# vision-agh/apse_uav

Hardware: AMD Instinct MI355X
Metric: 4K UAV frames/sec (whole node) (higher is better)
Workload: dtype f32

## Files before the change

### apse_uav_amd/_lib.py

```python
import ctypes as C
import os

import numpy as np

_HERE = os.path.dirname(os.path.abspath(__file__))
LIB_PATH = os.environ.get("APSE_HIP_LIB") or os.path.join(_HERE, "libapse_hip.so")

APSE_OK = 0


class ApseError(RuntimeError):
    pass


class Config(C.Structure):
    _fields_ = [
        ("struct_size", C.c_int), ("device", C.c_int), ("max_batch", C.c_int),
        ("frame_h", C.c_int), ("frame_w", C.c_int), ("image_h", C.c_int), ("image_w", C.c_int),
        ("blocks", C.c_int * 4), ("num_classes", C.c_int),
        ("score_thresh", C.c_float), ("box_nms", C.c_float), ("rpn_nms", C.c_float), ("mask_thresh", C.c_float),
        ("rpn_pre_topk", C.c_int), ("rpn_post_topk", C.c_int), ("dets_per_image", C.c_int),
        ("pixel_mean", C.c_float * 3), ("assoc_roi", C.c_int), ("embed_dim", C.c_int), ("assoc_scale", C.c_float),
        ("compute_dtype", C.c_int), ("storage16", C.c_int),
    ]


class ConfigArch(Config):
    _fields_ = [("arch", C.c_int)]


class ResultsLayout(C.Structure):
    _fields_ = [("bytes", C.c_size_t), ("n_max", C.c_int), ("dets_per_image", C.c_int), ("embed_dim", C.c_int),
                ("max_batch", C.c_int)] + [(k, C.c_size_t) for k in (
                    "total", "offset", "prop_count", "img", "cls", "roi", "score", "box_resized", "box", "valid", "rect",
                    "mass", "centroid", "closest", "embedding")]


class RenderItem(C.Structure):
    _fields_ = [("image", C.c_int), ("rect", C.c_int * 4), ("words_per_row", C.c_int), ("bits", C.c_void_p),
                ("box", C.c_float * 4), ("rgb", C.c_uint8 * 4), ("label_off", C.c_int), ("label_len", C.c_int)]


class MotsWindow(C.Structure):
    _fields_ = [("rect", C.c_int * 4), ("words_per_row", C.c_int), ("area", C.c_int), ("bits", C.c_void_p)]


class MotsObject(C.Structure):
    _fields_ = [("rect", C.c_int * 4), ("words_per_row", C.c_int), ("score", C.c_float), ("bits", C.c_void_p)]


class ConvDesc(C.Structure):
    _fields_ = [(k, C.c_int) for k in ("B", "H", "W", "Cin", "Cout", "KH", "KW", "stride", "pad", "relu", "res_mode",
                                       "cfg", "splitk", "prec", "fuse_reduce", "x_st", "res_st", "y_st")]


_lib = None


def load():
    global _lib
    if _lib is not None:
        return _lib
    if not os.path.exists(LIB_PATH):
        raise ApseError("libapse_hip.so not found at %s: build it with `python -c 'import __graft_entry__ as g; g.build()'` "
                        "or `make -C apse_uav_amd/csrc` (there is no CPU fallback)" % LIB_PATH)
    import torch
    lib = C.CDLL(LIB_PATH)
    vp, i, f, sz = C.c_void_p, C.c_int, C.c_float, C.c_size_t
    sig = {
        "apse_create": ([C.POINTER(Config), C.POINTER(vp)], i),
        "apse_destroy": ([vp], None),
        "apse_last_error": ([vp], C.c_char_p),
        "apse_version": ([], C.c_char_p),
        "apse_set_weight": ([vp, C.c_char_p, vp, C.POINTER(C.c_int64), i], i),
        "apse_finalize_weights": ([vp], i),
        "apse_set_resize_tables": ([vp, vp, vp, i, vp, vp, i], i),
        "apse_set_camera": ([vp, C.POINTER(C.c_double), C.POINTER(C.c_double), i, vp, i, i], i),
        "apse_preprocess_frames": ([vp, vp, i, vp], i),
        "apse_preprocess_images": ([vp, vp, i, vp], i),
        "apse_backbone": ([vp, i, vp], i),
        "apse_rpn": ([vp, i, vp], i),
        "apse_rpn_levels": ([vp, i, i, vp], i),
        "apse_box_head": ([vp, i, vp], i),
        "apse_set_detections": ([vp, vp, vp, vp, vp, i, vp], i),
        "apse_mask_tail": ([vp, i, vp], i),
        "apse_embed": ([vp, i, vp], i),
        "apse_forward": ([vp, i, vp], i),
        "apse_results_describe": ([vp, C.POINTER(ResultsLayout)], i),
        "apse_read_results": ([vp, vp, sz, vp], i),
        "apse_read_results_begin": ([vp, vp, sz, vp], i),
        "apse_read_results_end": ([vp, vp], i),
        "apse_copy_mask_window": ([vp, i, i, i, i, i, vp, vp], i),
        "apse_copy_mask_windows": ([vp, i, vp, vp, vp, vp, vp], i),
        "apse_host_copy": ([vp, vp, sz, i], i),
        "apse_feature_shape": ([vp, C.c_char_p, C.POINTER(C.c_int * 3)], i),
        "apse_export_feature": ([vp, C.c_char_p, vp, i, vp], i),
        "apse_debug_tensor": ([vp, C.c_char_p, vp, sz, C.POINTER(sz), vp], i),
        "apse_flops": ([vp, i, C.c_double, C.c_double], C.c_double),
        "apse_profile": ([vp, i], i),
        "apse_profile_read": ([vp, C.POINTER(C.c_double * 42), i], i),
        "apse_conv_packed_elems": ([C.POINTER(ConvDesc)], sz),
        "apse_conv_pack_weight": ([C.POINTER(ConvDesc), vp, i, vp, vp], i),
        "apse_conv2d": ([C.POINTER(ConvDesc), vp, vp, vp, vp, vp, vp, sz, vp], i),
        "apse_maxpool3x3s2": ([vp, vp, i, i, i, i, vp], i),
        "apse_maxpool3x3s2_typed": ([vp, vp, i, i, i, i, i, vp], i),
        "apse_roi_align": ([C.POINTER(vp), C.POINTER(i), C.POINTER(i), vp, i, i, i, vp, vp], i),
        "apse_roi_align_typed": ([C.POINTER(vp), C.POINTER(i), C.POINTER(i), vp, i, i, i, i, vp, vp], i),
        "apse_roi_pool": ([vp, i, i, vp, vp, i, i, f, vp, vp], i),
        "apse_roi_features": ([vp, i, vp, vp, i, i, vp, vp], i),
        "apse_nms_rank": ([vp, vp, vp, i, i, i, i, f, i, vp, vp, vp, vp, vp], i),
        "apse_mask_centroid_dense": ([vp, i, i, C.POINTER(C.c_int * 3), vp], i),
        "apse_mask_closest_dense": ([vp, i, i, f, f, C.POINTER(C.c_int * 2), vp], i),
        "apse_l2_normalize": ([vp, vp, i, i, vp], i),
        "apse_sqdist": ([vp, vp, i, i, i, vp, vp], i),
        "apse_undistort_gamma": ([vp, vp, i, i, i, C.POINTER(C.c_double), C.POINTER(C.c_double), i, vp, i, i, vp], i),
        "apse_lab_tables_host": ([vp, vp, C.c_size_t], C.c_size_t),
        "apse_replay_create": ([i, i, f, i], vp),
        "apse_replay_destroy": ([vp], None),
        "apse_replay_step": ([vp, i, i, vp, vp, vp, C.c_char_p, i, vp], i),
        "apse_replay_packed": ([vp, vp, C.c_longlong, i, i, i, vp, C.c_longlong], C.c_longlong),
        "apse_replay_max_id": ([vp], i),
        "apse_replay_next_id": ([vp], i),
        "apse_render_workspace_bytes": ([i, i, i], sz),
        "apse_render_instances": ([vp, vp, i, i, i, i, vp, i, vp, sz, vp, i, vp, sz, vp], i),
        "apse_render_pack_mask": ([vp, i, i, vp, vp], i),
        "apse_render_font_host": ([vp, sz], sz),
        "apse_mots_split_workspace_bytes": ([], sz),
        "apse_mots_split_idmap": ([vp, i, i, i, vp, sz, vp, vp, vp, vp, sz, vp], i),
        "apse_mots_rle_to_bits": ([vp, vp, i, i, i, vp, vp], i),
        "apse_mots_overlaps": ([vp, i, vp, i, vp, i, vp, vp], i),
        "apse_mots_render_idmap": ([vp, vp, i, i, i, vp, vp], i),
        "apse_resize_normalize": ([vp, vp, vp, vp, vp, vp, i, vp, vp, i, i, i, i, i, i, i, i, C.POINTER(f * 3), vp], i),
        "apse_assoc_fc_workspace_bytes": ([i, i, i], sz),
        "apse_assoc_fc_forward": ([vp, vp, vp, i, i, i, vp, vp, vp, sz, vp], i),
        "apse_assoc_fc_backward": ([vp, vp, vp, vp, i, i, i, vp, vp, vp, sz, vp], i),
        "apse_triplet_workspace_bytes": ([i], sz),
        "apse_triplet_hard_forward": ([vp, vp, i, i, f, i, vp, vp, sz, vp], i),
        "apse_triplet_all_forward": ([vp, vp, i, i, f, i, vp, vp, sz, vp], i),
        "apse_triplet_hard_backward": ([vp, i, i, i, vp, vp, vp, vp], i),
        "apse_triplet_all_backward": ([vp, i, i, i, vp, vp, vp, vp], i),
        "apse_sgd_step": ([vp, vp, vp, C.c_longlong, f, f, f, f, i, i, vp], i),
        "apse_coco_box_iou": ([vp, vp, vp, i, i, i, vp, vp, vp, vp, vp], i),
        "apse_coco_poly_to_bits": ([vp, vp, i, vp, i, vp, vp, vp, i, vp, vp, vp, vp], i),
        "apse_coco_match": ([vp, vp, vp, i, i, i, vp, vp, vp, i, vp, vp, vp, i, vp, i, vp, i, vp, vp, vp, vp, vp], i),
        "apse_coco_accumulate_workspace_bytes": ([C.c_longlong], sz),
        "apse_coco_sort_lists": ([vp, vp, i, vp, C.c_longlong, i, vp, vp, sz, vp], i),
        "apse_coco_accumulate": ([vp, vp, vp, i, vp, i, vp, vp, vp, C.c_longlong, i, vp, i, i, i, i, i, vp, vp, vp, vp, sz,
                                  vp], i),
        "apse_mask_roi_features": ([vp, i, vp, i, vp, vp], i),
        "apse_mask_train_workspace_bytes": ([i, i], sz),
        "apse_mask_pack_elems": ([i, i, i, i], sz),
        "apse_mask_pack_weight": ([vp, vp, i, i, i, i, i, vp, vp, vp], i),
        "apse_mask_conv_forward": ([vp, vp, vp, i, i, i, i, i, i, i, i, i, i, i, vp, vp, sz, vp], i),
        "apse_mask_conv3x3": ([vp, vp, vp, i, i, vp, vp], i),
        "apse_mask_relu_grad": ([vp, vp, C.c_longlong, vp, vp], i),
        "apse_mask_bias_grad": ([vp, C.c_longlong, vp, vp, sz, vp], i),
        "apse_mask_wgrad": ([vp, vp, i, i, vp, vp, sz, vp], i),
        "apse_mask_loss_forward": ([vp, i, vp, vp, i, vp, vp, sz, vp], i),
        "apse_mask_loss_backward": ([vp, i, vp, vp, i, vp, vp, vp], i),
        "apse_mask_predictor_backward": ([vp, vp, vp, vp, i, i, vp, vp, vp, vp, sz, vp], i),
    }
    for name, (args, ret) in sig.items():
        fn = getattr(lib, name)
        fn.argtypes = args
        fn.restype = ret
    _lib = lib
    return lib


EXPORTS = ["apse_create", "apse_destroy", "apse_last_error", "apse_version", "apse_set_weight", "apse_finalize_weights",
           "apse_set_resize_tables", "apse_set_camera", "apse_preprocess_frames", "apse_preprocess_images", "apse_backbone", "apse_rpn", "apse_rpn_levels",
           "apse_box_head", "apse_set_detections", "apse_mask_tail", "apse_embed", "apse_forward", "apse_results_describe",
           "apse_read_results", "apse_read_results_begin", "apse_read_results_end", "apse_copy_mask_window", "apse_copy_mask_windows", "apse_host_copy", "apse_feature_shape", "apse_export_feature", "apse_debug_tensor",
           "apse_flops", "apse_profile", "apse_profile_read", "apse_conv_packed_elems", "apse_conv_pack_weight", "apse_conv2d", "apse_maxpool3x3s2",
           "apse_maxpool3x3s2_typed", "apse_roi_align", "apse_roi_align_typed", "apse_roi_pool", "apse_roi_features", "apse_nms_rank", "apse_mask_centroid_dense", "apse_mask_closest_dense",
           "apse_l2_normalize", "apse_sqdist", "apse_undistort_gamma", "apse_lab_tables_host", "apse_resize_normalize", "apse_replay_create", "apse_replay_destroy",
           "apse_replay_step", "apse_replay_packed", "apse_replay_max_id", "apse_replay_next_id", "apse_render_workspace_bytes",
           "apse_render_instances", "apse_render_pack_mask", "apse_render_font_host", "apse_mots_split_workspace_bytes",
           "apse_mots_split_idmap", "apse_mots_rle_to_bits", "apse_mots_overlaps", "apse_mots_render_idmap",
           "apse_assoc_fc_workspace_bytes", "apse_assoc_fc_forward", "apse_assoc_fc_backward", "apse_triplet_workspace_bytes",
           "apse_triplet_hard_forward", "apse_triplet_all_forward", "apse_triplet_hard_backward", "apse_triplet_all_backward",
           "apse_sgd_step", "apse_coco_box_iou", "apse_coco_poly_to_bits", "apse_coco_match",
           "apse_coco_accumulate_workspace_bytes", "apse_coco_sort_lists", "apse_coco_accumulate",
           "apse_mask_roi_features", "apse_mask_train_workspace_bytes", "apse_mask_pack_elems", "apse_mask_pack_weight",
           "apse_mask_conv_forward", "apse_mask_conv3x3", "apse_mask_relu_grad", "apse_mask_bias_grad", "apse_mask_wgrad", "apse_mask_loss_forward",
           "apse_mask_loss_backward", "apse_mask_predictor_backward"]


def stream_ptr():
    import torch
    return C.c_void_p(torch.cuda.current_stream().cuda_stream)


def check(rc, ctx=None, what=""):
    if rc != APSE_OK:
        msg = load().apse_last_error(ctx).decode() if ctx is not None else ""
        raise ApseError("%s failed (code %d) %s" % (what, rc, msg))


def ptr(t):
    if t is None:
        return C.c_void_p(0)
    if isinstance(t, np.ndarray):
        assert t.flags["C_CONTIGUOUS"]
        return C.c_void_p(t.ctypes.data)
    assert t.is_contiguous()
    return C.c_void_p(t.data_ptr())
```

### apse_uav_amd/csrc/conv_winograd.hip

```cpp
#include "apse_common.h"

namespace {
constexpr int WTR = 16, WTC = 4;
constexpr int WT = WTR * WTC;
constexpr int WN = 64;
constexpr int KC = 8;
constexpr int NTHR = 512;
constexpr int SLICE_F = 16 * WT * KC;
constexpr size_t WINO_LDS = (size_t)2 * 2 * SLICE_F * sizeof(float);
static_assert(WN == WT, "V and U slices share one size");
static_assert((size_t)16 * WT * 32 * sizeof(float) <= WINO_LDS, "epilogue chunk must fit the staging LDS");
}

__global__ __launch_bounds__(NTHR) void conv_winograd_f32(const ConvParams p) {
    extern __shared__ __attribute__((aligned(16))) char smem[];
    float* Vs = reinterpret_cast<float*>(smem);
    float* Us = Vs + 2 * SLICE_F;
    float* Cs = reinterpret_cast<float*>(smem);

    const int tid = threadIdx.x;
    const int lane = tid & 63, wave = tid >> 6;
    const int fr = lane & 31, fh = lane >> 5;

    const int tiles_y = (p.OH + 2 * WTR - 1) / (2 * WTR), tiles_x = (p.OW + 2 * WTC - 1) / (2 * WTC);
    const int nblk = p.Cout / WN;
    const int nwg = p.B * tiles_y * tiles_x * nblk;
    int bid;
    {
        const int wg = blockIdx.x;
        const int q = nwg >> 3, r = nwg & 7, xcd = wg & 7, idx = wg >> 3;
        bid = (xcd < r ? xcd * (q + 1) : r * (q + 1) + (xcd - r) * q) + idx;
    }
    const int nb = bid % nblk;
    int rest = bid / nblk;
    const int bx = rest % tiles_x; rest /= tiles_x;
    const int by = rest % tiles_y;
    const int b = rest / tiles_y;
    const int oy0 = by * 2 * WTR, ox0 = bx * 2 * WTC, n0 = nb * WN;
    const int C = 1 << p.cin_log2;
    const int nsteps = C / KC;

    const int cg = tid & 1, t = (tid >> 1) & (WT - 1), ti = tid >> 7;
    const int ra = ti == 0 ? 0 : (ti == 2 ? 2 : 1);
    const int rb = ti == 0 ? 2 : (ti == 1 ? 2 : (ti == 2 ? 1 : 3));
    const int iy_a = oy0 + 2 * (t / WTC) - 1 + ra, iy_b = oy0 + 2 * (t / WTC) - 1 + rb;
    const int ix0 = ox0 + 2 * (t % WTC) - 1;
    const __amdgpu_buffer_rsrc_t xrsrc =
        __builtin_amdgcn_make_buffer_rsrc(const_cast<float*>(p.x), 0, (int)((((unsigned)(p.B * p.H * p.W)) << p.cin_log2) * 4u), 0x00020000);
    unsigned xoff[2][4];
#pragma unroll
    for (int r = 0; r < 2; ++r) {
        const int iy = r ? iy_b : iy_a;
#pragma unroll
        for (int c = 0; c < 4; ++c) {
            const int ix = ix0 + c;
            const bool in = (unsigned)iy < (unsigned)p.H && (unsigned)ix < (unsigned)p.W;
            xoff[r][c] = in ? ((((unsigned)((b * p.H + iy) * p.W + ix)) << p.cin_log2) + (unsigned)(cg * 4)) * 4u : 0x80000000u;
        }
    }
    const float* ubase = p.wu + (size_t)n0 * KC;
    const size_t ustep = (size_t)16 * p.Cout * KC;

    f32x4 xr[2][4], ur[4];
    auto fetch = [&](int s) {
        const unsigned kb = (unsigned)(s * KC * 4);
#pragma unroll
        for (int r = 0; r < 2; ++r)
#pragma unroll
            for (int c = 0; c < 4; ++c)
                xr[r][c] = __builtin_bit_cast(f32x4, __builtin_amdgcn_raw_buffer_load_b128(xrsrc, (int)(xoff[r][c] + kb), 0, 0));
        const float* us = ubase + (size_t)s * ustep;
#pragma unroll
        for (int k = 0; k < 4; ++k) {
            const int q = tid + NTHR * k;
            const int xi = q >> 7, co = (q >> 1) & 63, h = q & 1;
            ur[k] = *reinterpret_cast<const f32x4*>(us + ((size_t)xi * p.Cout + co) * KC + h * 4);
        }
    };
    auto stage = [&](int buf) {
        f32x4 x[4];
#pragma unroll
        for (int c = 0; c < 4; ++c) x[c] = ti == 1 ? xr[0][c] + xr[1][c] : xr[0][c] - xr[1][c];
        const f32x4 v[4] = {x[0] - x[2], x[1] + x[2], x[2] - x[1], x[1] - x[3]};
        const int sw = (cg ^ ((t >> 3) & 1)) * 4;
#pragma unroll
        for (int j = 0; j < 4; ++j)
            *reinterpret_cast<f32x4*>(Vs + buf * SLICE_F + ((4 * ti + j) * WT + t) * KC + sw) = v[j];
#pragma unroll
        for (int k = 0; k < 4; ++k) {
            const int q = tid + NTHR * k;
            const int xi = q >> 7, co = (q >> 1) & 63, h = q & 1;
            *reinterpret_cast<f32x4*>(Us + buf * SLICE_F + (xi * WN + co) * KC + ((h ^ ((co >> 3) & 1)) * 4)) = ur[k];
        }
    };

    f32x16 acc[2][2][2];
#pragma unroll
    for (int a = 0; a < 2; ++a)
#pragma unroll
        for (int i = 0; i < 2; ++i)
#pragma unroll
            for (int j = 0; j < 2; ++j)
#pragma unroll
                for (int v = 0; v < 16; ++v) acc[a][i][j][v] = 0.f;

    fetch(0);
    stage(0);
    __syncthreads();
    const int fsw = (fh ^ ((fr >> 3) & 1)) * 4;
    for (int s = 0; s < nsteps; ++s) {
        const int buf = s & 1;
        const bool more = s + 1 < nsteps;
        if (more) fetch(s + 1);
#pragma unroll
        for (int a = 0; a < 2; ++a) {
            const int xi = 2 * wave + a;
            f32x4 af[2], bf[2];
#pragma unroll
            for (int i = 0; i < 2; ++i) af[i] = *reinterpret_cast<const f32x4*>(Vs + buf * SLICE_F + (xi * WT + 32 * i + fr) * KC + fsw);
#pragma unroll
            for (int j = 0; j < 2; ++j) bf[j] = *reinterpret_cast<const f32x4*>(Us + buf * SLICE_F + (xi * WN + 32 * j + fr) * KC + fsw);
#pragma unroll
            for (int k = 0; k < 4; ++k)
#pragma unroll
                for (int i = 0; i < 2; ++i)
#pragma unroll
                    for (int j = 0; j < 2; ++j)
                        acc[a][i][j] = __builtin_amdgcn_mfma_f32_32x32x2f32(af[i][k], bf[j][k], acc[a][i][j], 0, 0, 0);
        }
        if (more) stage(buf ^ 1);
        __syncthreads();
    }

    const int et = tid >> 3, eg = tid & 7;
    const int oy = oy0 + 2 * (et / WTC), ox = ox0 + 2 * (et % WTC);
    typedef unsigned u32x4_t __attribute__((ext_vector_type(4)));
#pragma unroll
    for (int j = 0; j < 2; ++j) {
#pragma unroll
        for (int a = 0; a < 2; ++a)
#pragma unroll
            for (int i = 0; i < 2; ++i)
#pragma unroll
                for (int v = 0; v < 16; ++v) {
                    const int row = 32 * i + (v & 3) + 8 * (v >> 2) + 4 * fh;
                    Cs[((2 * wave + a) * WT + row) * 32 + fr] = acc[a][i][j][v];
                }
        __syncthreads();
        f32x4 m[16];
#pragma unroll
        for (int k = 0; k < 16; ++k) m[k] = *reinterpret_cast<const f32x4*>(Cs + (k * WT + et) * 32 + eg * 4);
        f32x4 s0[4], s1[4];
#pragma unroll
        for (int c = 0; c < 4; ++c) {
            s0[c] = m[c] + m[4 + c] + m[8 + c];
            s1[c] = m[4 + c] - m[8 + c] - m[12 + c];
        }
        const int co = n0 + 32 * j + 4 * eg;
        const f32x4 bias4 = p.bias ? *reinterpret_cast<const f32x4*>(p.bias + co) : f32x4{0.f, 0.f, 0.f, 0.f};
        f32x4 y[2][2] = {{s0[0] + s0[1] + s0[2], s0[1] - s0[2] - s0[3]}, {s1[0] + s1[1] + s1[2], s1[1] - s1[2] - s1[3]}};
#pragma unroll
        for (int dy = 0; dy < 2; ++dy)
#pragma unroll
            for (int dx = 0; dx < 2; ++dx) {
                f32x4 val = y[dy][dx] + bias4;
                if (p.relu) {
#pragma unroll
                    for (int k = 0; k < 4; ++k) val[k] = apse_relu(val[k]);
                }
                if (oy + dy < p.OH && ox + dx < p.OW)
                    APSE_NT_STORE(val, reinterpret_cast<f32x4*>(p.y + ((size_t)(b * p.OH + oy + dy) * p.OW + ox + dx) * p.y_ld + p.y_coff + co));
            }
        __syncthreads();
    }
}

bool apse_conv_winograd_ok(const ConvParams& p, int max_items) {
    return p.prec == 0 && p.x_st == 0 && p.y_st == 0 && p.KH == 3 && p.KW == 3 && p.stride == 1 && p.pad == 1 && p.out_mode == 0 &&
           p.res_mode == 0 && p.splitk == 1 && p.Cout % WN == 0 && p.cin_log2 >= 3 && p.OH == p.H && p.OW == p.W &&
           (p.y_ld & 3) == 0 && (p.y_coff & 3) == 0 && ((((size_t)max_items * p.H * p.W) << p.cin_log2) * 4 < 0x7fff0000ull);
}

int apse_conv_winograd_blocks(const ConvParams& p) {
    return ((p.OH + 2 * WTR - 1) / (2 * WTR)) * ((p.OW + 2 * WTC - 1) / (2 * WTC)) * (p.Cout / WN);
}

int apse_launch_conv_winograd(const ConvParams& p, hipStream_t s, hipEvent_t ev0, hipEvent_t ev1) {
    if (!p.wu || !apse_conv_winograd_ok(p, p.B) || p.m_count) return APSE_E_INVALID;
    static bool attr_done = false;
    if (!attr_done) {
        hipFuncSetAttribute(reinterpret_cast<const void*>(&conv_winograd_f32), hipFuncAttributeMaxDynamicSharedMemorySize, (int)WINO_LDS);
        attr_done = true;
    }
    const int tiles_y = (p.OH + 2 * WTR - 1) / (2 * WTR), tiles_x = (p.OW + 2 * WTC - 1) / (2 * WTC);
    const int grid = p.B * tiles_y * tiles_x * (p.Cout / WN);
    if (ev0) hipEventRecord(ev0, s);
    hipLaunchKernelGGL(conv_winograd_f32, dim3(grid), dim3(NTHR), WINO_LDS, s, p);
    if (ev1) hipEventRecord(ev1, s);
    return hipGetLastError() == hipSuccess ? APSE_OK : APSE_E_HIP;
}
```

### apse_uav_amd/csrc/detector.hip

```cpp
#include "apse_common.h"
#include "../../include/apse_hip.h"
#include "preproc_pixel.h"

#include <math.h>
#include <stdio.h>
#include <string.h>

#include <map>
#include <mutex>
#include <string>
#include <vector>

struct RpnLevel { const float* head; int H, W, stride; int n; int k; float base[3][4]; };
struct RpnLevels { RpnLevel lv[5]; int head_ld; int pre_topk; };
struct TopkJob { int kind; int level; int begin, count; int nsrc; int src[4]; int src_count[4]; int dst; int dst_count; };
struct FpnMaps { const void* p[4]; int H[4], W[4]; float scale[4]; int st; };
struct PasteParams {
    const float* boxes; const int* cls; const int* total; const float* logits; int M, ldc; float sx, sy; int out_h, out_w;
    int words_per_row; float thresh; float* boxes_out; int* valid; int* rect; uint64_t* bits; unsigned long long* sums;
};
extern "C" {
int apse_k_pil_resize(const uint8_t*, uint8_t*, void*, int, uint8_t*, const int*, const int*, int, const int*, const int*, int, int,
                      int, int, int, int, int, int, const float*, const UndistortParams*, const LabTables*, const void*, const int*, int, hipStream_t);
int apse_k_undistort_build_map_compact(const UndistortParams*, void*, int*, hipStream_t);
// ... 1531 lines not shown
    if (bytes) *bytes = n;
    if (!dst) return APSE_OK;
    if (n > max_bytes) return fail(c, APSE_E_INVALID, "debug buffer too small for " + nm);
    HIPCHK(c, hipMemcpyAsync(dst, src, n, hipMemcpyDeviceToDevice, (hipStream_t)stream));
    return APSE_OK;
}

double apse_flops(apse_ctx* c, int batch, double proposals, double detections) {
    if (!c || !c->finalized) return 0.0;
    double f = 0;
    for (auto& s : c->backbone) if (s.kind == S_CONV || s.kind == S_BNECK) f += s.c.flops_per_item * batch;
    for (auto& s : c->rpnhead) f += s.c.flops_per_item * batch;
    for (auto& s : c->c4_res5box) f += s.c.flops_per_item * proposals;
    for (auto& s : c->boxhead) f += s.c.flops_per_item * proposals;
    for (auto& s : c->maskhead) f += s.c.flops_per_item * detections;
    for (auto& s : c->embedfc) f += s.c.flops_per_item * detections;
    return f;
}

size_t apse_conv_packed_elems(const apse_conv_desc* d) {
    const int cin_p = pow2_at_least(d->Cin);
    return (size_t)apse_roundup(d->Cout, 128) * d->KH * apse_roundup(d->KW * cin_p, 32);
}

int apse_conv_pack_weight(const apse_conv_desc* d, const float* w, int cin_real, const float* scale, float* packed) {
    if (!d || !w || !packed) return APSE_E_INVALID;
    const int cin_p = pow2_at_least(d->Cin);
    const int KWCp = apse_roundup(d->KW * cin_p, 32);
    memset(packed, 0, apse_conv_packed_elems(d) * sizeof(float));
    pack_oihw(w, d->Cout, cin_real, d->KH, d->KW, cin_p, scale, packed, KWCp);
    return APSE_OK;
}

int apse_conv2d(const apse_conv_desc* d, const float* x, const float* w, const float* bias, const float* res, float* y, float* ws,
                size_t ws_bytes, void* stream) {
    if (!d || !x || !w || !y) return APSE_E_INVALID;
    const int cin_p = pow2_at_least(d->Cin);
    if (cin_p != d->Cin) return APSE_E_INVALID;
    ConvParams p;
    memset(&p, 0, sizeof p);
    p.x = x; p.w = w; p.bias = bias; p.res = res; p.y = y; p.ws = ws;
    p.B = d->B; p.H = d->H; p.W = d->W; p.cin_log2 = apse_ilog2(cin_p);
    p.KH = d->KH; p.KW = d->KW; p.stride = d->stride; p.pad = d->pad;
    p.KWCp = apse_roundup(d->KW * cin_p, 32);
    p.OH = (d->H + 2 * d->pad - d->KH) / d->stride + 1;
    p.OW = (d->W + 2 * d->pad - d->KW) / d->stride + 1;
    p.Cout = d->Cout; p.relu = d->relu; p.res_mode = d->res_mode;
    p.M = p.B * p.OH * p.OW; p.m_per_item = p.OH * p.OW;
    p.y_ld = d->Cout; p.steps_total = p.KH * (p.KWCp / 32);
    p.prec = (d->prec == 1 || d->prec == 2) ? d->prec : 0;
    p.x_st = d->x_st; p.res_st = d->res_st; p.y_st = d->y_st;
    if (p.x_st < 0 || p.x_st > 2 || p.res_st < 0 || p.res_st > 2 || p.y_st < 0 || p.y_st > 2) return APSE_E_INVALID;
    if (p.prec && p.x_st && p.x_st != p.prec) return APSE_E_INVALID;
    if (p.x_st && cin_p < 8) return APSE_E_INVALID;
    int sk = 1;
    int cfg = apse_conv_pick_cfg(p.M, p.Cout, p.steps_total, &sk);
    if (d->cfg >= 0) { cfg = d->cfg; sk = 1; p.no_stream = (d->cfg != APSE_CFG_STREAM && d->cfg != APSE_CFG_GLDS && d->cfg != APSE_CFG_SKINNY); }
    if (d->splitk > 0) sk = d->splitk;
    if (sk > p.steps_total) sk = p.steps_total;
    p.splitk = sk;
    if (sk > 1 && (size_t)sk * p.M * p.Cout * sizeof(float) > ws_bytes) return APSE_E_INVALID;
    if (sk > 1 && d->fuse_reduce) {
        static int* cnt = nullptr;
        if (!cnt) { if (hipMalloc(reinterpret_cast<void**>(&cnt), 65536 * sizeof(int)) != hipSuccess) return APSE_E_NOMEM; hipMemset(cnt, 0, 65536 * sizeof(int)); }
        p.tile_cnt = cnt;
    }
    if (!p.prec) return apse_launch_conv(p, cfg, (hipStream_t)stream);
    const size_t ne = (size_t)apse_roundup(p.Cout, 128) * p.KH * p.KWCp;
    static uint16_t* d16 = nullptr;
    static size_t d16_cap = 0;
    if (ne > d16_cap) {
        hipDeviceSynchronize();
        if (d16) hipFree(d16);
        d16 = nullptr; d16_cap = 0;
        if (hipMalloc(reinterpret_cast<void**>(&d16), ne * 2) != hipSuccess) return APSE_E_NOMEM;
        d16_cap = ne;
    }
    int rc = apse_k_round16(w, d16, ne, p.prec, (hipStream_t)stream);
    if (rc) return rc;
    p.w16 = d16;
    return apse_launch_conv(p, cfg, (hipStream_t)stream);
}

int apse_maxpool3x3s2(const float* x, float* y, int B, int H, int W, int C, void* stream) {
    return apse_k_maxpool3x3s2(x, y, B, H, W, C, 0, (hipStream_t)stream);
}

int apse_maxpool3x3s2_typed(const void* x, void* y, int B, int H, int W, int C, int storage, void* stream) {
    if (!x || !y || B < 1 || H < 1 || W < 1 || C < 4 || (C & 3) || storage < 0 || storage > 2) return APSE_E_INVALID;
    return apse_k_maxpool3x3s2(x, y, B, H, W, C, storage, (hipStream_t)stream);
}

static int roi_align_stateless(const void* const* feats, const int* hs, const int* ws, const float* rois, int n, int per_img,
                               int out_size, int st, void* out, void* stream) {
    if (!feats || !hs || !ws || !rois || !out || n < 0 || out_size < 1 || st < 0 || st > 2) return APSE_E_INVALID;
    FpnMaps F;
    static const float sc[4] = {0.25f, 0.125f, 0.0625f, 0.03125f};
    for (int l = 0; l < 4; ++l) { F.p[l] = feats[l]; F.H[l] = hs[l]; F.W[l] = ws[l]; F.scale[l] = sc[l]; }
    F.st = st;
    static int* total_dev = nullptr;
    if (!total_dev) hipMalloc(reinterpret_cast<void**>(&total_dev), sizeof(int));
    hipMemcpyAsync(total_dev, &n, sizeof(int), hipMemcpyHostToDevice, (hipStream_t)stream);
    hipStreamSynchronize((hipStream_t)stream);
    std::vector<int> img(n);
    for (int i = 0; i < n; ++i) img[i] = per_img > 0 ? i / per_img : 0;
    int* img_dev = nullptr;
    if (hipMalloc(reinterpret_cast<void**>(&img_dev), sizeof(int) * (n > 0 ? n : 1)) != hipSuccess) return APSE_E_NOMEM;
    hipMemcpy(img_dev, img.data(), sizeof(int) * n, hipMemcpyHostToDevice);
    int rc = apse_k_roi_align(&F, rois, img_dev, nullptr, total_dev, 0, n, out_size, out, st, (hipStream_t)stream);
    hipStreamSynchronize((hipStream_t)stream);
    hipFree(img_dev);
    return rc;
}

int apse_roi_align(const float* const* feats, const int* hs, const int* ws, const float* rois, int n, int per_img, int out_size,
                   float* out, void* stream) {
    return roi_align_stateless(reinterpret_cast<const void* const*>(feats), hs, ws, rois, n, per_img, out_size, 0, out, stream);
}

int apse_roi_align_typed(const void* const* feats, const int* hs, const int* ws, const float* rois, int n, int per_img,
                         int out_size, int storage, void* out, void* stream) {
    return roi_align_stateless(feats, hs, ws, rois, n, per_img, out_size, storage, out, stream);
}

int apse_roi_pool(const float* feat, int H, int W, const float* rois, const int* roi_img, int n, int out_size, float scale,
                  float* out, void* stream) {
    static int* total_dev = nullptr;
    if (!total_dev) hipMalloc(reinterpret_cast<void**>(&total_dev), sizeof(int));
    hipMemcpyAsync(total_dev, &n, sizeof(int), hipMemcpyHostToDevice, (hipStream_t)stream);
    hipStreamSynchronize((hipStream_t)stream);
    return apse_k_roi_pool(feat, 0, H, W, rois, roi_img, total_dev, n, out_size, scale, out, 0, 0, (hipStream_t)stream);
}

int apse_nms_rank(const float* boxes, const float* scores, const int* valid, int n, int cat_div, int cat_mod, int ncat, float thr,
                  int topk, float* out_boxes, float* out_scores, int* out_index, int* out_count, void* stream) {
    if (ncat < 1 || ncat > 8 || n > 8192) return APSE_E_INVALID;
    hipStream_t s = (hipStream_t)stream;
    int *keep_idx = nullptr, *keep_cnt = nullptr;
    uint32_t* maxc = nullptr;
    if (hipMalloc(reinterpret_cast<void**>(&keep_idx), sizeof(int) * 8 * NMS_SLOT) != hipSuccess) return APSE_E_NOMEM;
    hipMalloc(reinterpret_cast<void**>(&keep_cnt), sizeof(int) * 8);
    hipMalloc(reinterpret_cast<void**>(&maxc), sizeof(uint32_t));
    std::vector<float> hb((size_t)n * 4);
    std::vector<int> hv(n);
    hipMemcpy(hb.data(), boxes, hb.size() * 4, hipMemcpyDeviceToHost);
    hipMemcpy(hv.data(), valid, hv.size() * 4, hipMemcpyDeviceToHost);
    float m = 0.f;
    bool any = false;
    for (int i = 0; i < n; ++i)
        if (hv[i]) for (int k = 0; k < 4; ++k) { m = (!any || hb[i * 4 + k] > m) ? hb[i * 4 + k] : m; any = true; }
    uint32_t mb;
    memcpy(&mb, &m, 4);
    hipMemcpy(maxc, &mb, 4, hipMemcpyHostToDevice);
    void* scratch = nullptr;
    if (hipMalloc(&scratch, apse_nms_scratch_bytes(8)) != hipSuccess) return APSE_E_NOMEM;
    int rc = apse_k_nms_percat(boxes, scores, valid, n, cat_div, cat_mod, maxc, thr, keep_idx, keep_cnt, ncat, scratch, 0, 1, 0, s);
    if (!rc) rc = apse_k_rank_final(boxes, scores, n, keep_idx, keep_cnt, ncat, topk, out_boxes, out_scores, out_index, out_count, nullptr, 1, s);
    hipStreamSynchronize(s);
    hipFree(keep_idx); hipFree(keep_cnt); hipFree(maxc); hipFree(scratch);
    return rc;
}

static int dense_scratch(int H, int W, uint64_t** bits, unsigned long long** sums) {
    static uint64_t* b = nullptr;
    static unsigned long long* sm = nullptr;
    static size_t words = 0;
// ... 152 lines not shown
```

### include/apse_hip.h

```cpp
#ifndef APSE_HIP_H
#define APSE_HIP_H
#include <stddef.h>
#include <stdint.h>
#ifdef __cplusplus
extern "C" {
#endif

#define APSE_OK 0
#define APSE_E_INVALID (-1)
#define APSE_E_HIP (-2)
#define APSE_E_NOMEM (-3)
#define APSE_E_STATE (-4)
#define APSE_E_MISSING (-5)

typedef struct apse_ctx apse_ctx;

#define APSE_MAX_CLASSES 80
#define APSE_C4_MAX_PRE_TOPK 6000
#define APSE_C4_MAX_BATCH 2
#define APSE_MAX_FRAME_W 49152
#define APSE_MAX_FRAME_H 32768
typedef struct apse_config {
    int struct_size;
    int device;
// ... 16 lines not shown
    int compute_dtype;
    int storage16;
    int arch;
} apse_config;

typedef struct apse_results_layout {
    size_t bytes;
    int n_max, dets_per_image, embed_dim, max_batch;
    size_t total;
    size_t offset;
    size_t prop_count;
    size_t img;
    size_t cls;
    size_t roi;
    size_t score;
    size_t box_resized;
    size_t box;
    size_t valid;
    size_t rect;
    size_t mass;
    size_t centroid;
    size_t closest;
    size_t embedding;
} apse_results_layout;

int apse_create(const apse_config* cfg, apse_ctx** out);
void apse_destroy(apse_ctx* ctx);
const char* apse_last_error(apse_ctx* ctx);
const char* apse_version(void);

int apse_set_weight(apse_ctx* ctx, const char* name, const float* host, const int64_t* shape, int ndim);
int apse_finalize_weights(apse_ctx* ctx);

int apse_set_resize_tables(apse_ctx* ctx, const int* hbounds, const int* hcoef, int hksize, const int* vbounds,
                           const int* vcoef, int vksize);

int apse_set_camera(apse_ctx* ctx, const double* m9, const double* dist, int ndist, const uint8_t* lut256_host, int do_undistort,
                    int do_gamma);

int apse_preprocess_frames(apse_ctx* ctx, const uint8_t* frames_dev, int batch, void* stream);
int apse_preprocess_images(apse_ctx* ctx, const float* images_dev, int batch, void* stream);
int apse_backbone(apse_ctx* ctx, int batch, void* stream);
int apse_rpn(apse_ctx* ctx, int batch, void* stream);
int apse_rpn_levels(apse_ctx* ctx, int batch, int level_mask, void* stream);
int apse_box_head(apse_ctx* ctx, int batch, void* stream);
int apse_set_detections(apse_ctx* ctx, const float* boxes_host, const int* classes_host, const float* scores_host,
                        const int* counts_host, int batch, void* stream);
int apse_mask_tail(apse_ctx* ctx, int batch, void* stream);
int apse_embed(apse_ctx* ctx, int batch, void* stream);
int apse_roi_features(apse_ctx* ctx, int image, const float* rois_dev, const uint8_t* masks_dev, int n, int roi_size,
                      float* out_dev, void* stream);
int apse_forward(apse_ctx* ctx, int batch, void* stream);

int apse_results_describe(apse_ctx* ctx, apse_results_layout* out);
int apse_read_results(apse_ctx* ctx, void* host_dst, size_t bytes, void* stream);
int apse_read_results_begin(apse_ctx* ctx, void* host_dst, size_t bytes, void* stream);
int apse_read_results_end(apse_ctx* ctx, void* host_dst);
int apse_copy_mask_window(apse_ctx* ctx, int det, int x0, int y0, int x1, int y1, uint64_t* dst_dev, void* stream);
int apse_copy_mask_windows(apse_ctx* ctx, int n, const int* dets_host, const int* rects_host, uint64_t* dst_dev,
                           const long long* dst_word_offsets_host, void* stream);
int apse_feature_shape(apse_ctx* ctx, const char* name, int* chw3);
int apse_export_feature(apse_ctx* ctx, const char* name, float* dst_nchw_dev, int batch, void* stream);
int apse_debug_tensor(apse_ctx* ctx, const char* name, void* dst_dev, size_t max_bytes, size_t* bytes, void* stream);
double apse_flops(apse_ctx* ctx, int batch, double proposals, double detections);

int apse_profile(apse_ctx* ctx, int enable);
int apse_profile_read(apse_ctx* ctx, double* out42, int reset);

typedef struct apse_conv_desc {
    int B, H, W, Cin;
    int Cout, KH, KW, stride, pad;
    int relu;
    int res_mode;
    int cfg;
    int splitk;
    int prec;
    int fuse_reduce;
    int x_st, res_st, y_st;
} apse_conv_desc;
size_t apse_conv_packed_elems(const apse_conv_desc* d);
int apse_conv_pack_weight(const apse_conv_desc* d, const float* w_oihw, int cin_real, const float* scale, float* packed);
int apse_conv2d(const apse_conv_desc* d, const float* x_dev, const float* w_packed_dev, const float* bias_dev,
                const float* res_dev, float* y_dev, float* ws_dev, size_t ws_bytes, void* stream);
int apse_maxpool3x3s2(const float* x_dev, float* y_dev, int B, int H, int W, int C, void* stream);
int apse_maxpool3x3s2_typed(const void* x_dev, void* y_dev, int B, int H, int W, int C, int storage, void* stream);
int apse_roi_align(const float* const* feats_dev, const int* hs, const int* ws, const float* rois_dev, int n, int per_img,
                   int out_size, float* out_dev, void* stream);
int apse_roi_align_typed(const void* const* feats_dev, const int* hs, const int* ws, const float* rois_dev, int n, int per_img,
                         int out_size, int storage, void* out_dev, void* stream);
int apse_roi_pool(const float* feat_dev, int H, int W, const float* rois_dev, const int* roi_img_dev, int n, int out_size,
                  float scale, float* out_dev, void* stream);
int apse_nms_rank(const float* boxes_dev, const float* scores_dev, const int* valid_dev, int n, int cat_div, int cat_mod,
                  int ncat, float thr, int topk, float* out_boxes_dev, float* out_scores_dev, int* out_index_dev,
                  int* out_count_dev, void* stream);
int apse_mask_centroid_dense(const uint8_t* mask_dev, int H, int W, int* out_xy_mass_host3, void* stream);
int apse_mask_closest_dense(const uint8_t* mask_dev, int H, int W, float px, float py, int* out_xy_host2, void* stream);
int apse_l2_normalize(const float* x_dev, float* y_dev, int n, int D, void* stream);
int apse_sqdist(const float* a_dev, const float* b_dev, int O, int N, int D, float* out_dev, void* stream);
int apse_undistort_gamma(const uint8_t* src_dev, uint8_t* dst_dev, int B, int H, int W, const double* mtx3x3_host,
                         const double* dist_host, int ndist, const uint8_t* lut256_host, int do_undistort, int do_gamma,
                         void* stream);
size_t apse_lab_tables_host(const uint8_t* lut256_host, void* out, size_t cap);
int apse_resize_normalize(const uint8_t* frames_dev, uint8_t* tmp_dev, float* out_nhwc4_dev, uint8_t* resized_u8_dev,
                          const int* hb_dev, const int* hc_dev, int hk, const int* vb_dev, const int* vc_dev, int vk, int B,
                          int H, int W, int OH, int OW, int PH, int PW, const float* mean3_host, void* stream);

typedef struct apse_replay apse_replay;
apse_replay* apse_replay_create(int host_id, int embed_dim, float dist_thresh, int max_unseen_frames);
void apse_replay_destroy(apse_replay* r);
int apse_replay_step(apse_replay* r, int frame_idx, int n, const float* emb_host, const int* centroid_host,
                     const int* closest_host, char* line_out, int line_cap, int* det_ids_out);
long long apse_replay_packed(apse_replay* r, const float* records_host, long long total_floats, int nrec, int dets_per_image,
                             int first_frame, char* lines_out, long long cap);
int apse_replay_max_id(const apse_replay* r);
int apse_replay_next_id(const apse_replay* r);


int apse_host_copy(void* dst, const void* src, size_t bytes, int threads);

#define APSE_RENDER_MAX_ITEMS 1024
#define APSE_RENDER_MAX_BREAKS 64
#define APSE_RENDER_MAX_LINES 4
typedef struct apse_render_item {
    int image;
    int rect[4];
    int words_per_row;
    const uint64_t* bits;
    float box[4];
    uint8_t rgb[4];
    int label_off, label_len;
} apse_render_item;
size_t apse_render_workspace_bytes(int H, int W, int n);
int apse_render_instances(const uint8_t* frames_dev, uint8_t* out_dev, int B, int H, int W, int bgr,
                          const apse_render_item* items_dev, int n, const uint8_t* labels_dev, size_t label_bytes,
                          const float* scale_breaks_host, int nbreaks, void* ws_dev, size_t ws_bytes, void* stream);
int apse_render_pack_mask(const uint8_t* mask_dev, int H, int W, uint64_t* words_dev, void* stream);
size_t apse_render_font_host(uint8_t* out, size_t cap);

#define APSE_MOTS_MAX_OBJECTS 1024
#define APSE_MOTS_MAX_PAIRS 65536
#define APSE_MOTS_MAX_UNION 1024
typedef struct apse_mots_window {
    int rect[4];
    int words_per_row;
    int area;
    uint64_t* bits;
} apse_mots_window;
typedef struct apse_mots_object {
    int rect[4];
    int words_per_row;
    float score;
    const uint64_t* bits;
} apse_mots_object;
size_t apse_mots_split_workspace_bytes(void);
int apse_mots_split_idmap(const uint16_t* idmap, int H, int W, int max_values, uint64_t* pool, size_t pool_words, int* values,
                          apse_mots_window* windows, int* info, void* ws, size_t ws_bytes, void* stream);
int apse_mots_rle_to_bits(const int* ends, const int* ends_off, int n, int h, int w, const apse_mots_window* windows,
                          void* stream);
int apse_mots_overlaps(const apse_mots_window* windows, int n_windows, const int* pairs, int npairs, const int* union_idx,
                       int n_union, int* out, void* stream);
int apse_mots_render_idmap(const apse_mots_object* objects, const int* values_host, int n, int H, int W, uint16_t* idmap,
                           void* stream);

#define APSE_COCO_MAX_GROUPS (1 << 24)
#define APSE_COCO_MAX_GT 4096
#define APSE_COCO_MAX_DET 4096
// ... 73 lines not shown
```

Baseline: 185.5.

## Software-pipeline Winograd conv main loop with interleaved loads and MFMA groups

Result: faster. 193.9 (median of 6 runs) (+4.5%).

```diff
diff --git a/apse_uav_amd/_lib.py b/apse_uav_amd/_lib.py
--- a/apse_uav_amd/_lib.py
+++ b/apse_uav_amd/_lib.py
@@ -4,7 +4,9 @@
 import numpy as np
 
 _HERE = os.path.dirname(os.path.abspath(__file__))
-LIB_PATH = os.environ.get("APSE_HIP_LIB") or os.path.join(_HERE, "libapse_hip.so")
+_TREE_LIB = os.path.join(_HERE, "libapse_hip.so")
+LIB_PATH = os.environ.get("APSE_HIP_LIB") or _TREE_LIB
+TOOL_ENTRIES = ("apse_winograd_pack_filter", "apse_winograd_conv2d")
 
 APSE_OK = 0
 
@@ -102,6 +104,8 @@
         "apse_conv_packed_elems": ([C.POINTER(ConvDesc)], sz),
         "apse_conv_pack_weight": ([C.POINTER(ConvDesc), vp, i, vp, vp], i),
         "apse_conv2d": ([C.POINTER(ConvDesc), vp, vp, vp, vp, vp, vp, sz, vp], i),
+        "apse_winograd_pack_filter": ([vp, i, i, vp], i),
+        "apse_winograd_conv2d": ([C.POINTER(ConvDesc), vp, vp, vp, vp, vp], i),
         "apse_maxpool3x3s2": ([vp, vp, i, i, i, i, vp], i),
         "apse_maxpool3x3s2_typed": ([vp, vp, i, i, i, i, i, vp], i),
         "apse_roi_align": ([C.POINTER(vp), C.POINTER(i), C.POINTER(i), vp, i, i, i, vp, vp], i),
@@ -161,6 +165,8 @@
         "apse_mask_predictor_backward": ([vp, vp, vp, vp, i, i, vp, vp, vp, vp, sz, vp], i),
     }
     for name, (args, ret) in sig.items():
+        if name in TOOL_ENTRIES and LIB_PATH != _TREE_LIB and not hasattr(lib, name):
+            continue
         fn = getattr(lib, name)
         fn.argtypes = args
         fn.restype = ret
@@ -172,7 +178,7 @@
            "apse_set_resize_tables", "apse_set_camera", "apse_preprocess_frames", "apse_preprocess_images", "apse_backbone", "apse_rpn", "apse_rpn_levels",
            "apse_box_head", "apse_set_detections", "apse_mask_tail", "apse_embed", "apse_forward", "apse_results_describe",
            "apse_read_results", "apse_read_results_begin", "apse_read_results_end", "apse_copy_mask_window", "apse_copy_mask_windows", "apse_host_copy", "apse_feature_shape", "apse_export_feature", "apse_debug_tensor",
-           "apse_flops", "apse_profile", "apse_profile_read", "apse_conv_packed_elems", "apse_conv_pack_weight", "apse_conv2d", "apse_maxpool3x3s2",
+           "apse_flops", "apse_profile", "apse_profile_read", "apse_conv_packed_elems", "apse_conv_pack_weight", "apse_conv2d", "apse_winograd_pack_filter", "apse_winograd_conv2d", "apse_maxpool3x3s2",
            "apse_maxpool3x3s2_typed", "apse_roi_align", "apse_roi_align_typed", "apse_roi_pool", "apse_roi_features", "apse_nms_rank", "apse_mask_centroid_dense", "apse_mask_closest_dense",
            "apse_l2_normalize", "apse_sqdist", "apse_undistort_gamma", "apse_lab_tables_host", "apse_resize_normalize", "apse_replay_create", "apse_replay_destroy",
            "apse_replay_step", "apse_replay_packed", "apse_replay_max_id", "apse_replay_next_id", "apse_render_workspace_bytes",
diff --git a/apse_uav_amd/csrc/conv_winograd.hip b/apse_uav_amd/csrc/conv_winograd.hip
--- a/apse_uav_amd/csrc/conv_winograd.hip
+++ b/apse_uav_amd/csrc/conv_winograd.hip
@@ -6,6 +6,7 @@
 constexpr int WN = 64;
 constexpr int KC = 8;
 constexpr int NTHR = 512;
+constexpr int G_U = 1, G_ROWS = 2, G_V = 3;
 constexpr int SLICE_F = 16 * WT * KC;
 constexpr size_t WINO_LDS = (size_t)2 * 2 * SLICE_F * sizeof(float);
 static_assert(WN == WT, "V and U slices share one size");
@@ -19,7 +20,7 @@
     float* Cs = reinterpret_cast<float*>(smem);
 
     const int tid = threadIdx.x;
-    const int lane = tid & 63, wave = tid >> 6;
+    const int lane = tid & 63, wave = __builtin_amdgcn_readfirstlane(tid >> 6);
     const int fr = lane & 31, fh = lane >> 5;
 
     const int tiles_y = (p.OH + 2 * WTR - 1) / (2 * WTR), tiles_x = (p.OW + 2 * WTC - 1) / (2 * WTC);
@@ -40,13 +41,15 @@
     const int C = 1 << p.cin_log2;
     const int nsteps = C / KC;
 
-    const int cg = tid & 1, t = (tid >> 1) & (WT - 1), ti = tid >> 7;
+    const int cg = tid & 1, t = (tid >> 1) & (WT - 1), ti = wave >> 1;
     const int ra = ti == 0 ? 0 : (ti == 2 ? 2 : 1);
     const int rb = ti == 0 ? 2 : (ti == 1 ? 2 : (ti == 2 ? 1 : 3));
+    const float sgn = ti == 1 ? 1.f : -1.f;
     const int iy_a = oy0 + 2 * (t / WTC) - 1 + ra, iy_b = oy0 + 2 * (t / WTC) - 1 + rb;
     const int ix0 = ox0 + 2 * (t % WTC) - 1;
     const __amdgpu_buffer_rsrc_t xrsrc =
         __builtin_amdgcn_make_buffer_rsrc(const_cast<float*>(p.x), 0, (int)((((unsigned)(p.B * p.H * p.W)) << p.cin_log2) * 4u), 0x00020000);
+    const __amdgpu_buffer_rsrc_t xnone = __builtin_amdgcn_make_buffer_rsrc(const_cast<float*>(p.x), 0, 0, 0x00020000);
     unsigned xoff[2][4];
 #pragma unroll
     for (int r = 0; r < 2; ++r) {
@@ -58,40 +61,48 @@
             xoff[r][c] = in ? ((((unsigned)((b * p.H + iy) * p.W + ix)) << p.cin_log2) + (unsigned)(cg * 4)) * 4u : 0x80000000u;
         }
     }
-    const float* ubase = p.wu + (size_t)n0 * KC;
-    const size_t ustep = (size_t)16 * p.Cout * KC;
+    const __amdgpu_buffer_rsrc_t ursrc =
+        __builtin_amdgcn_make_buffer_rsrc(const_cast<float*>(p.wu), 0, (int)((((unsigned)(16 * p.Cout)) << p.cin_log2) * 4u), 0x00020000);
+    const unsigned ustep = (unsigned)(16 * p.Cout * KC * 4);
+    unsigned uoff[4], ulds[4];
+#pragma unroll
+    for (int k = 0; k < 4; ++k) {
+        const int q = tid + NTHR * k;
+        const int xi = q >> 7, co = (q >> 1) & 63, h = q & 1;
+        uoff[k] = (unsigned)(((xi * p.Cout + n0 + co) * KC + h * 4) * 4);
+        ulds[k] = (unsigned)((xi * WN + co) * KC + ((h ^ ((co >> 3) & 1)) * 4));
+    }
+    const int vlds = (4 * ti * WT + t) * KC + (cg ^ ((t >> 3) & 1)) * 4;
 
     f32x4 xr[2][4], ur[4];
-    auto fetch = [&](int s) {
+    auto fetch_u = [&](int s) {
+        const unsigned kb = (unsigned)s * ustep;
+#pragma unroll
+        for (int k = 0; k < 4; ++k) ur[k] = __builtin_bit_cast(f32x4, __builtin_amdgcn_raw_buffer_load_b128(ursrc, (int)(uoff[k] + kb), 0, 0));
+    };
+    auto fetch_x = [&](int s) {
         const unsigned kb = (unsigned)(s * KC * 4);
+        const __amdgpu_buffer_rsrc_t rs = s < nsteps ? xrsrc : xnone;
 #pragma unroll
         for (int r = 0; r < 2; ++r)
 #pragma unroll
             for (int c = 0; c < 4; ++c)
-                xr[r][c] = __builtin_bit_cast(f32x4, __builtin_amdgcn_raw_buffer_load_b128(xrsrc, (int)(xoff[r][c] + kb), 0, 0));
-        const float* us = ubase + (size_t)s * ustep;
-#pragma unroll
-        for (int k = 0; k < 4; ++k) {
-            const int q = tid + NTHR * k;
-            const int xi = q >> 7, co = (q >> 1) & 63, h = q & 1;
-            ur[k] = *reinterpret_cast<const f32x4*>(us + ((size_t)xi * p.Cout + co) * KC + h * 4);
-        }
-    };
-    auto stage = [&](int buf) {
-        f32x4 x[4];
-#pragma unroll
-        for (int c = 0; c < 4; ++c) x[c] = ti == 1 ? xr[0][c] + xr[1][c] : xr[0][c] - xr[1][c];
-        const f32x4 v[4] = {x[0] - x[2], x[1] + x[2], x[2] - x[1], x[1] - x[3]};
-        const int sw = (cg ^ ((t >> 3) & 1)) * 4;
-#pragma unroll
-        for (int j = 0; j < 4; ++j)
-            *reinterpret_cast<f32x4*>(Vs + buf * SLICE_F + ((4 * ti + j) * WT + t) * KC + sw) = v[j];
-#pragma unroll
-        for (int k = 0; k < 4; ++k) {
-            const int q = tid + NTHR * k;
-            const int xi = q >> 7, co = (q >> 1) & 63, h = q & 1;
-            *reinterpret_cast<f32x4*>(Us + buf * SLICE_F + (xi * WN + co) * KC + ((h ^ ((co >> 3) & 1)) * 4)) = ur[k];
-        }
+                xr[r][c] = __builtin_bit_cast(f32x4, __builtin_amdgcn_raw_buffer_load_b128(rs, (int)(xoff[r][c] + kb), 0, 0));
+    };
+    auto write_u = [&](int buf) {
+#pragma unroll
+        for (int k = 0; k < 4; ++k) *reinterpret_cast<f32x4*>(Us + buf * SLICE_F + ulds[k]) = ur[k];
+    };
+    auto xform_rows = [&]() {
+#pragma unroll
+        for (int c = 0; c < 4; ++c)
+#pragma unroll
+            for (int e = 0; e < 4; ++e) xr[0][c][e] = __builtin_fmaf(xr[1][c][e], sgn, xr[0][c][e]);
+    };
+    auto write_v = [&](int buf) {
+        const f32x4 v[4] = {xr[0][0] - xr[0][2], xr[0][1] + xr[0][2], xr[0][2] - xr[0][1], xr[0][1] - xr[0][3]};
+#pragma unroll
+        for (int j = 0; j < 4; ++j) *reinterpret_cast<f32x4*>(Vs + buf * SLICE_F + vlds + j * WT * KC) = v[j];
     };
 
     f32x16 acc[2][2][2];
@@ -104,32 +115,50 @@
 #pragma unroll
                 for (int v = 0; v < 16; ++v) acc[a][i][j][v] = 0.f;
 
-    fetch(0);
-    stage(0);
+    fetch_u(0);
+    fetch_x(0);
+    write_u(0);
+    xform_rows();
+    write_v(0);
+    __builtin_amdgcn_sched_barrier(0);
+    fetch_u(1);
+    __builtin_amdgcn_sched_barrier(0);
+    fetch_x(1);
     __syncthreads();
     const int fsw = (fh ^ ((fr >> 3) & 1)) * 4;
+    const int frag = (2 * wave * WT + fr) * KC + fsw;
+    f32x4 af[2][2], bf[2][2];
+    auto read_frags = [&](int buf, int a) {
+#pragma unroll
+        for (int i = 0; i < 2; ++i) af[a][i] = *reinterpret_cast<const f32x4*>(Vs + buf * SLICE_F + frag + (a * WT + 32 * i) * KC);
+#pragma unroll
+        for (int j = 0; j < 2; ++j) bf[a][j] = *reinterpret_cast<const f32x4*>(Us + buf * SLICE_F + frag + (a * WN + 32 * j) * KC);
+    };
+    auto mfma_group = [&](int a, int k) {
+#pragma unroll
+        for (int i = 0; i < 2; ++i)
+#pragma unroll
+            for (int j = 0; j < 2; ++j)
+                acc[a][i][j] = __builtin_amdgcn_mfma_f32_32x32x2f32(af[a][i][k], bf[a][j][k], acc[a][i][j], 0, 0, 0);
+    };
+    read_frags(0, 0);
     for (int s = 0; s < nsteps; ++s) {
         const int buf = s & 1;
-        const bool more = s + 1 < nsteps;
-        if (more) fetch(s + 1);
-#pragma unroll
-        for (int a = 0; a < 2; ++a) {
-            const int xi = 2 * wave + a;
-            f32x4 af[2], bf[2];
-#pragma unroll
-            for (int i = 0; i < 2; ++i) af[i] = *reinterpret_cast<const f32x4*>(Vs + buf * SLICE_F + (xi * WT + 32 * i + fr) * KC + fsw);
-#pragma unroll
-            for (int j = 0; j < 2; ++j) bf[j] = *reinterpret_cast<const f32x4*>(Us + buf * SLICE_F + (xi * WN + 32 * j + fr) * KC + fsw);
-#pragma unroll
-            for (int k = 0; k < 4; ++k)
-#pragma unroll
-                for (int i = 0; i < 2; ++i)
-#pragma unroll
-                    for (int j = 0; j < 2; ++j)
-                        acc[a][i][j] = __builtin_amdgcn_mfma_f32_32x32x2f32(af[i][k], bf[j][k], acc[a][i][j], 0, 0, 0);
+        read_frags(buf, 1);
+#pragma unroll
+        for (int g = 0; g < 7; ++g) {
+            __builtin_amdgcn_sched_barrier(0);
+            if (g == G_U) { write_u(buf ^ 1); fetch_u(s + 2); }
+            if (g == G_ROWS) xform_rows();
+            if (g == G_V) { write_v(buf ^ 1); fetch_x(s + 2); }
+            __builtin_amdgcn_sched_barrier(0);
+            mfma_group(g >> 2, g & 3);
         }
-        if (more) stage(buf ^ 1);
+        __builtin_amdgcn_sched_barrier(0);
         __syncthreads();
+        read_frags(buf ^ 1, 0);
+        __builtin_amdgcn_sched_barrier(0);
+        mfma_group(1, 3);
     }
 
     const int et = tid >> 3, eg = tid & 7;
diff --git a/apse_uav_amd/csrc/detector.hip b/apse_uav_amd/csrc/detector.hip
--- a/apse_uav_amd/csrc/detector.hip
+++ b/apse_uav_amd/csrc/detector.hip
@@ -1637,6 +1637,27 @@
     return apse_launch_conv(p, cfg, (hipStream_t)stream);
 }
 
+int apse_winograd_pack_filter(const float* w, int Cout, int Cin, float* packed) {
+    if (!w || !packed || Cout < 1 || Cin < 8 || pow2_at_least(Cin) != Cin) return APSE_E_INVALID;
+    const std::vector<float> u = winograd_filters(w, Cout, Cin, Cin);
+    memcpy(packed, u.data(), u.size() * sizeof(float));
+    return APSE_OK;
+}
+
+int apse_winograd_conv2d(const apse_conv_desc* d, const float* x, const float* wu, const float* bias, float* y, void* stream) {
+    if (!d || !x || !wu || !y || d->B < 1 || d->H < 1 || d->W < 1 || d->Cin < 8 || pow2_at_least(d->Cin) != d->Cin) return APSE_E_INVALID;
+    ConvParams p;
+    memset(&p, 0, sizeof p);
+    p.x = x; p.wu = wu; p.bias = bias; p.y = y;
+    p.B = d->B; p.H = d->H; p.W = d->W; p.cin_log2 = apse_ilog2(d->Cin);
+    p.KH = d->KH; p.KW = d->KW; p.stride = d->stride; p.pad = d->pad;
+    p.OH = d->H; p.OW = d->W; p.Cout = d->Cout; p.relu = d->relu;
+    p.M = p.B * p.OH * p.OW; p.m_per_item = p.OH * p.OW;
+    p.y_ld = d->Cout; p.splitk = 1;
+    p.res_mode = d->res_mode; p.prec = d->prec; p.x_st = d->x_st; p.y_st = d->y_st;
+    return apse_launch_conv_winograd(p, (hipStream_t)stream);
+}
+
 int apse_maxpool3x3s2(const float* x, float* y, int B, int H, int W, int C, void* stream) {
     return apse_k_maxpool3x3s2(x, y, B, H, W, C, 0, (hipStream_t)stream);
 }
diff --git a/include/apse_hip.h b/include/apse_hip.h
--- a/include/apse_hip.h
+++ b/include/apse_hip.h
@@ -122,6 +122,9 @@
 int apse_conv_pack_weight(const apse_conv_desc* d, const float* w_oihw, int cin_real, const float* scale, float* packed);
 int apse_conv2d(const apse_conv_desc* d, const float* x_dev, const float* w_packed_dev, const float* bias_dev,
                 const float* res_dev, float* y_dev, float* ws_dev, size_t ws_bytes, void* stream);
+int apse_winograd_pack_filter(const float* w_oihw, int Cout, int Cin, float* packed);
+int apse_winograd_conv2d(const apse_conv_desc* d, const float* x_dev, const float* wu_dev, const float* bias_dev, float* y_dev,
+                         void* stream);
 int apse_maxpool3x3s2(const float* x_dev, float* y_dev, int B, int H, int W, int C, void* stream);
 int apse_maxpool3x3s2_typed(const void* x_dev, void* y_dev, int B, int H, int W, int C, int storage, void* stream);
 int apse_roi_align(const float* const* feats_dev, const int* hs, const int* ws, const float* rois_dev, int n, int per_img,
```
